# elybrand/quantized_neural_networks

Measured on NVIDIA B200. Metric: quantized weights/s, full-network GPFQ pass, higher is better.
Workload: dtype f64

## Files before the change

quantized_neural_networks_b200/csrc/api.cu:

```cuda
#include <math.h>
#include <stdarg.h>
#include <stdlib.h>

#include <algorithm>
#include <cmath>

#include "common.cuh"

int dense_gram_path(gpfq_ctx *, const float *, const float *, int64_t, int64_t, int64_t, const float *, int64_t,
                    int64_t, int64_t, const double *, const int *, const int *, int, double *, int64_t, int64_t,
                    gpfq_stats *, const double *G1_pre = nullptr, const double *G2_pre = nullptr, const double *d_scales = nullptr,
                    int64_t u0 = 0);
int dense_stream_path(gpfq_ctx *, const float *, const float *, int64_t, int64_t, int64_t, const float *, int64_t,
                      int64_t, int64_t, const double *, const int *, const int *, int, double *, int64_t, int64_t,
                      gpfq_stats *, const double *d_scales, int64_t u0);
int dense_gram_only(gpfq_ctx *, const float *, const float *, int64_t, int64_t, int64_t, double *, double *);
bool dense_gram_uses_i8(gpfq_ctx *, int64_t, int64_t, bool);
int conv_supported_kk(int kk);
int conv_pick_chunks(gpfq_ctx *, int64_t, int, int64_t *, int, bool, int64_t part_rows = 0);
bool conv_specialised_kk(int kk);
int conv_gram_stage(gpfq_ctx *, int, ConvPtrs, bool, int64_t, int, int, int64_t, double *, bool, int);
int conv_finalize_stage(gpfq_ctx *, const double *, int, int, int, bool, double *);
int conv_sweep_stage(gpfq_ctx *, int, const double *, const float *, double *, int64_t, int64_t, int64_t, int,
                     const double *, const int *, const int *, int, int64_t, const double *);
// ... 69 lines not shown
    *out = b.p;
    return GPFQ_OK;
}

extern "C" int gpfq_version(void) { return GPFQ_VERSION; }

extern "C" int gpfq_create(int device, gpfq_ctx **out) {
    if (!out) return GPFQ_ERR_ARG;
    *out = nullptr;
    int ndev = 0;
    if (cudaGetDeviceCount(&ndev) != cudaSuccess || device < 0 || device >= ndev) {
        cudaGetLastError();
        return GPFQ_ERR_UNSUPPORTED;
    }
    cudaDeviceProp prop;
    if (cudaGetDeviceProperties(&prop, device) != cudaSuccess) return GPFQ_ERR_CUDA;
    if (prop.major != 10) return GPFQ_ERR_UNSUPPORTED;
    if (cudaSetDevice(device) != cudaSuccess) return GPFQ_ERR_CUDA;
    gpfq_ctx *ctx = new gpfq_ctx();
    ctx->device = device;
    ctx->sm_count = prop.multiProcessorCount;
    ctx->smem_optin = prop.sharedMemPerBlockOptin;
    bool ok = cudaStreamCreateWithFlags(&ctx->own_stream, cudaStreamNonBlocking) == cudaSuccess &&
              cudaStreamCreateWithFlags(&ctx->copy_stream, cudaStreamNonBlocking) == cudaSuccess;
    ctx->ring.resize(GPFQ_RING);
    for (auto &r : ctx->ring)
        for (int i = 0; ok && i < 8; ++i) ok = cudaEventCreate(&r.e[i]) == cudaSuccess;
    ctx->cur = &ctx->ring[0];
    for (int i = 0; ok && i < 4; ++i) ok = cudaEventCreateWithFlags(&ctx->ev_copy[i], cudaEventDisableTiming) == cudaSuccess;
    for (int i = 0; ok && i < 12; ++i) ok = cudaEventCreateWithFlags(&ctx->ev_chain[i], cudaEventDisableTiming) == cudaSuccess;
    for (int i = 0; ok && i < 8; ++i) ok = cudaStreamCreateWithFlags(&ctx->aux_stream[i], cudaStreamNonBlocking) == cudaSuccess;
    if (!ok) {
        delete ctx;
        return GPFQ_ERR_CUDA;
    }
    ctx->stream = ctx->own_stream;
    *out = ctx;
    return GPFQ_OK;
}

extern "C" int64_t gpfq_conv_partial_bytes(gpfq_ctx *ctx) { return ctx ? ctx->conv_part_bytes : 0; }

extern "C" int gpfq_trim(gpfq_ctx *ctx) {
    if (!ctx) return GPFQ_ERR_ARG;
    cudaSetDevice(ctx->device);
    cudaStreamSynchronize(ctx->stream);
    cudaStreamSynchronize(ctx->copy_stream);
    for (auto &s : ctx->aux_stream) if (s) cudaStreamSynchronize(s);
    for (auto &b : ctx->ws) {
        if (b.p) cudaFree(b.p);
        b.p = nullptr;
        b.cap = 0;
    }
    for (auto &b : ctx->pinned) {
        if (b.p) cudaFreeHost(b.p);
        b.p = nullptr;
        b.cap = 0;
    }
    ctx->alph_cache.clear();
    ctx->alph_used = 0;
    ctx->i8_oom_bytes = 0;
    return GPFQ_OK;
}

extern "C" void gpfq_destroy(gpfq_ctx *ctx) {
    if (!ctx) return;
    gpfq_trim(ctx);
    for (auto &r : ctx->ring)
        for (auto &e : r.e) if (e) cudaEventDestroy(e);
    for (auto &e : ctx->ev_copy) if (e) cudaEventDestroy(e);
    for (auto &e : ctx->ev_chain) if (e) cudaEventDestroy(e);
    for (auto &s : ctx->aux_stream) if (s) cudaStreamDestroy(s);
    if (ctx->own_stream) cudaStreamDestroy(ctx->own_stream);
    if (ctx->copy_stream) cudaStreamDestroy(ctx->copy_stream);
    delete ctx;
}

extern "C" const char *gpfq_last_error(const gpfq_ctx *ctx) { return ctx ? ctx->err.c_str() : "null context"; }

extern "C" int gpfq_set_option(gpfq_ctx *ctx, const char *key, int64_t value) {
    if (!ctx || !key) return GPFQ_ERR_ARG;
    ctx->err.clear();
    if (!strcmp(key, "gram_kernel")) {
        if (value < 0 || value > 2) return gpfq_fail(ctx, GPFQ_ERR_ARG, "gram_kernel must be 0, 1 or 2");
        ctx->gram_variant = (int)value;
    } else if (!strcmp(key, "i8_pairs_d")) {
        if (value != 0 && (value < 2 || value > 10)) return gpfq_fail(ctx, GPFQ_ERR_ARG, "i8_pairs_d must be 0 or 2..10");
        ctx->i8_pairs_d = (int)value;
    } else if (!strcmp(key, "corr_pack")) {
        if (value < 0 || value > 2) return gpfq_fail(ctx, GPFQ_ERR_ARG, "corr_pack must be 0, 1 or 2");
        ctx->corr_pack = (int)value;
    } else if (!strcmp(key, "corr_small")) {
        ctx->corr_direct_small = value != 0;
    } else if (!strcmp(key, "corr_rows")) {
        if (value != 0 && value != 4 && value != 6 && value != 8) return gpfq_fail(ctx, GPFQ_ERR_ARG, "corr_rows must be 0, 4, 6 or 8");
        ctx->corr_rb = (int)value;
    } else if (!strcmp(key, "corr_strip")) {
        if (value != 0 && value != 2) return gpfq_fail(ctx, GPFQ_ERR_ARG, "corr_strip must be 0 or 2");
        ctx->corr_strip = (int)value;
    } else if (!strcmp(key, "conv_kernel")) {
        if (value < 0 || value > 3) return gpfq_fail(ctx, GPFQ_ERR_ARG, "conv_kernel must be 0, 1, 2 or 3");
        ctx->conv_variant = (int)value;
    } else if (!strcmp(key, "sweep_outer")) {
        if (value < 0 || value > 3) return gpfq_fail(ctx, GPFQ_ERR_ARG, "sweep_outer must be 0, 1, 2 or 3");
        ctx->lowrank_variant = (int)value;
    } else if (!strcmp(key, "sweep_walk")) {
        if (value < 0 || value > 2) return gpfq_fail(ctx, GPFQ_ERR_ARG, "sweep_walk must be 0, 1 or 2");
        ctx->sweep_walk = (int)value;
    } else if (!strcmp(key, "sweep_i8")) {
        if (value < 0 || value > 2) return gpfq_fail(ctx, GPFQ_ERR_ARG, "sweep_i8 must be 0, 1 or 2");
        ctx->sweep_i8 = (int)value;
    } else {
        return gpfq_fail(ctx, GPFQ_ERR_ARG, "unknown option '%s'", key);
    }
    return GPFQ_OK;
}

extern "C" int gpfq_set_rounding(gpfq_ctx *ctx, int32_t mode, const uint64_t *seeds, int32_t n_seeds) {
    if (!ctx) return GPFQ_ERR_ARG;
    ctx->err.clear();
    if (mode == GPFQ_ROUND_NEAREST) {
        ctx->rounding = mode;
        ctx->seeds.clear();
        return GPFQ_OK;
    }
    if (mode != GPFQ_ROUND_STOCHASTIC) return gpfq_fail(ctx, GPFQ_ERR_ARG, "unknown rounding mode %d", mode);
    if (!seeds || n_seeds < 1) return gpfq_fail(ctx, GPFQ_ERR_ARG, "stochastic rounding needs n_seeds >= 1 seeds");
    ctx->rounding = mode;
    ctx->seeds.assign(seeds, seeds + n_seeds);
    return GPFQ_OK;
}

extern "C" int gpfq_set_stream(gpfq_ctx *ctx, void *cuda_stream) {
    if (!ctx) return GPFQ_ERR_ARG;
    cudaStream_t next = cuda_stream ? (cudaStream_t)cuda_stream : ctx->own_stream;
    if (next != ctx->stream) {
        cudaSetDevice(ctx->device);
        if (cudaStreamSynchronize(ctx->stream) != cudaSuccess) cudaGetLastError();
        ctx->stream = next;
    }
    return GPFQ_OK;
}

struct Alphabets {
    const double *d_levels = nullptr;
    const int *d_koff = nullptr;
    const int *d_flags = nullptr;
    std::vector<int> h_koff, h_flags;
};

static int alphabet_is_equispaced(const double *a, int K) {
    if (K < 2) return 0;
    const double step = (a[K - 1] - a[0]) / (K - 1);
    if (!(step > 0.0) || !std::isfinite(step)) return 0;
    for (int k = 0; k < K; ++k)
        if (!(fabs(a[k] - (a[0] + k * step)) <= 0.01 * step)) return 0;
    return 1;
}

static int upload_alphabets(gpfq_ctx *ctx, const double *alphabets, const int32_t *K, int n_alph, Alphabets *out) {
    if (!alphabets || !K || n_alph < 1 || n_alph > 1024) return gpfq_fail(ctx, GPFQ_ERR_ARG, "bad alphabet arguments");
    out->h_koff.assign(n_alph + 1, 0);
    for (int a = 0; a < n_alph; ++a) {
        if (K[a] < 1 || K[a] > GPFQ_MAX_K)
// ... 1070 lines not shown
```

quantized_neural_networks_b200/csrc/common.cuh:

```cuda
#pragma once
#include <cuda_runtime.h>
#include <stdint.h>
#include <stdio.h>
#include <string.h>

#include <string>
#include <vector>

#include "../../include/gpfq.h"

#define GPFQ_DEAD_NORM 1e-16
#define GPFQ_PERP_DOT 1e-10

struct DevBuf {
    void *p = nullptr;
    size_t cap = 0;
};

struct ConvPtrs {
    const float *const *Xp;
    const float *const *Xqp;
};

struct AlphEntry {
    std::vector<char> blob;
    size_t off = 0;
};

struct CallRecord {
    cudaEvent_t e[8] = {};
    bool rec[8] = {};
    int kind = 0;
    gpfq_stats st = {};
};
static constexpr int GPFQ_RING = 128;

struct gpfq_ctx {
    int device = 0;
    int sm_count = 148;
    size_t smem_optin = 0;
    cudaStream_t own_stream = nullptr;
    cudaStream_t copy_stream = nullptr;
    cudaStream_t stream = nullptr;
    std::vector<CallRecord> ring;
    int64_t calls = 0;
    CallRecord *cur = nullptr;
    cudaEvent_t ev_copy[4] = {};
    cudaStream_t aux_stream[8] = {};
    cudaEvent_t ev_chain[12] = {};
    std::string err = "";
    int launches = 0;
    int conv_variant = 0;
    int corr_pack = 0;
    bool corr_direct_small = false;
    int corr_occ[2][9] = {};
    int corr_rb = 0;
    int corr_strip_occ[2][2][3] = {};
    int corr_strip = 0;
    bool stream_literal = false;
    int gram_variant = 0;
    int lowrank_variant = 0;
    int sweep_walk = 0;
    int sweep_i8 = 0;
    int i8_pairs_d = 0;
    const double *h_alph = nullptr;
    const int *h_koff = nullptr, *h_flags = nullptr;
    int64_t conv_part_bytes = 0;
    double *gram_only_out = nullptr;
    int last_gram_kernel = 0;
    size_t i8_oom_bytes = 0;
    int rounding = GPFQ_ROUND_NEAREST;
    std::vector<uint64_t> seeds;
    const uint64_t *d_seeds = nullptr;
    DevBuf ws[48];
    DevBuf pinned[4];
    std::vector<AlphEntry> alph_cache;
    size_t alph_used = 0;
};

enum WsSlot {
    WS_X = 0, WS_XQ, WS_W, WS_Q, WS_WT, WS_QT, WS_G1, WS_G2, WS_PART, WS_DT, WS_NRM, WS_ALPH,
    WS_U, WS_PTRS, WS_CG, WS_CPART, WS_PATCH_A, WS_PATCH_B, WS_ACT_A, WS_ACT_B, WS_QIDX, WS_MISC,
    WS_I8_SQ, WS_I8_SX, WS_I8_E, WS_I8_TILES, WS_LR_XD, WS_LR_XT, WS_LR_U, WS_CORR_B,
    WS_SL_W, WS_SL_XT, WS_SL_XQT, WS_SL_XQ, WS_SL_U, WS_SL_KQ, WS_SL_E,
    WS_TC_TAB, WS_TC_G2S, WS_TC_G1S, WS_TC_E, WS_TC_P, WS_TC_W, WS_TC_G1M, WS_SCALES, WS_UNIT_H, WS_SEEDS
};

int gpfq_fail(gpfq_ctx *ctx, int code, const char *fmt, ...);
cudaError_t gpfq_record(gpfq_ctx *ctx, int which, cudaStream_t s);
int gpfq_ws(gpfq_ctx *ctx, int slot, size_t bytes, void **out);
int gpfq_pinned(gpfq_ctx *ctx, int slot, size_t bytes, void **out);

#define CUDA_TRY(ctx, expr)                                                                    \
    do {                                                                                       \
        cudaError_t _e = (expr);                                                               \
        if (_e != cudaSuccess)                                                                 \
            return gpfq_fail((ctx), _e == cudaErrorMemoryAllocation ? GPFQ_ERR_OOM : GPFQ_ERR_CUDA, \
                             "%s failed: %s (%s:%d)", #expr, cudaGetErrorString(_e), __FILE__, __LINE__); \
    } while (0)

#define GPFQ_TRY(expr)                \
    do {                              \
        int _rc = (expr);             \
        if (_rc != GPFQ_OK) return _rc; \
    } while (0)

#define KERNEL_CHECK(ctx)                                                                     \
    do {                                                                                      \
        (ctx)->launches++;                                                                    \
        cudaError_t _e = cudaGetLastError();                                                  \
        if (_e != cudaSuccess)                                                                \
            return gpfq_fail((ctx), GPFQ_ERR_CUDA, "kernel launch failed: %s (%s:%d)",        \
                             cudaGetErrorString(_e), __FILE__, __LINE__);                     \
    } while (0)

static constexpr int64_t CONV_PART_LIMIT = (int64_t)1 << 30;

static inline int64_t ceil_div64(int64_t a, int64_t b) { return (a + b - 1) / b; }

__device__ __forceinline__ double gpfq_bit_round(double v, const double *__restrict__ alph, int K) {
    double best = alph[0];
    double bd = fabs(__dsub_rn(best, v));
#pragma unroll 4
    for (int k = 1; k < K; ++k) {
        const double a = alph[k];
        const double d = fabs(__dsub_rn(a, v));
        if (d < bd) { bd = d; best = a; }
// ... 178 lines not shown
```

quantized_neural_networks_b200/csrc/slgemm_i8.cu:

```cuda
#include <algorithm>

#include "slgemm_i8.cuh"

namespace slg {
constexpr int TM = 128, TN = 64, BK = 64;
constexpr int STAGES = 3;
constexpr int S = 5;
constexpr int P_BITS = 8 * S - 2;
constexpr int A_SLICE = TM * BK, B_SLICE = TN * BK;
constexpr int STAGE_BYTES = S * (A_SLICE + B_SLICE);
constexpr int THREADS = 192;
constexpr int MAX_PHASES = 8;
constexpr int OUT_PITCH = TN + 1;
constexpr int KB_MAX = 408;
constexpr size_t SMEM = (size_t)STAGES * STAGE_BYTES + 1024  + 256  + TN * sizeof(double);
}

struct SlSeg {
    int SA, SB, D;
    int a_row0, b_row0;
    int k0, k0b, kblocks;
    double alpha;
    const double *row_mul;
    const int32_t *eA;
    int eA_const;
    const int8_t *A, *B;
    int64_t rowsA, rowsB;
};

struct SlArgs {
    SlSeg seg[2];
    int nseg, tiles_n;
    const int32_t *eB;
    int eB_const, b_row0;
    double *C;
    int64_t ldc;
    int M, N;
    int accumulate, vec2;
    int batch_rows_a, batch_rows_b, batch_k0a, batch_k0b;
    int64_t batch_c;
    int lower_only;
    int ktri;
};

__device__ __forceinline__ uint64_t umma_desc_sw64(uint32_t saddr) {
    return (uint64_t)((saddr & 0x3FFFFu) >> 4) | ((uint64_t)1 << 16) | ((uint64_t)(512 >> 4) << 32) | ((uint64_t)1 << 46) |
           ((uint64_t)4 << 61);
}

template <int SA, int SB, int D>
__device__ __forceinline__ void sl_issue_kblock(uint32_t tmem_base, uint64_t da, uint64_t db, uint32_t idesc, bool first) {
    using namespace slg;
#pragma unroll
    for (int d = 2; d <= D; ++d) {
        constexpr int dummy = 0;
        (void)dummy;
        const int k_lo = (d - SB) > 1 ? (d - SB) : 1, k_hi = SA < (d - 1) ? SA : (d - 1);
#pragma unroll
        for (int k = k_lo; k <= k_hi; ++k)
#pragma unroll
            for (int ks = 0; ks < BK / 32; ++ks)
                i8g::umma_i8(tmem_base + (uint32_t)((d - 2) * TN), da + (uint64_t)(((k - 1) * A_SLICE + ks * 32) >> 4),
                             db + (uint64_t)(((d - k - 1) * B_SLICE + ks * 32) >> 4), idesc,
                             (k == k_lo && ks == 0) ? (first ? 0u : 1u) : 1u);
    }
}

template <bool ROWMUL>
__global__ void __launch_bounds__(slg::THREADS, 1)
slgemm_i8_kernel(const SlArgs args) {
    using namespace i8g;
    using namespace slg;
    extern __shared__ unsigned char sl_smem_raw[];
    unsigned char *smem = reinterpret_cast<unsigned char *>(((uintptr_t)sl_smem_raw + 1023) & ~(uintptr_t)1023);
    uint64_t *full = reinterpret_cast<uint64_t *>(smem + (size_t)STAGES * STAGE_BYTES);
    uint64_t *empty = full + STAGES;
    uint64_t *seg_full = empty + STAGES;
    uint64_t *seg_empty = seg_full + 1;
    uint32_t *tmem_slot = reinterpret_cast<uint32_t *>(seg_empty + 1);
    double *colscale = reinterpret_cast<double *>(smem + (size_t)STAGES * STAGE_BYTES + 256);

    const int warp = threadIdx.x >> 5, lane = threadIdx.x & 31;
    const int ti = blockIdx.x / args.tiles_n, tj = blockIdx.x % args.tiles_n;
    if (args.lower_only && tj * TN > ti * TM + TM - 1) return;
    const int brow_a = (int)blockIdx.y * args.batch_rows_a, brow_b = (int)blockIdx.y * args.batch_rows_b;
    const int bk0a = (int)blockIdx.y * args.batch_k0a, bk0b = (int)blockIdx.y * args.batch_k0b;
    const int kcap = args.ktri ? tj + 1 : (1 << 30);

    if (threadIdx.x == 0) {
        for (int s = 0; s < STAGES; ++s) { mbar_init(&full[s], 1); mbar_init(&empty[s], 1); }
        mbar_init(seg_full, 1);
        mbar_init(seg_empty, 4);
        asm volatile("fence.mbarrier_init.release.cluster;\n" ::: "memory");
    }
    if (warp == 1) {
        asm volatile("tcgen05.alloc.cta_group::1.sync.aligned.shared::cta.b32 [%0], %1;\n" ::"r"(smem_u32(tmem_slot)), "r"(512));
        asm volatile("tcgen05.relinquish_alloc_permit.cta_group::1.sync.aligned;\n");
    }
    if (warp >= 2 && threadIdx.x - 64 < TN) {
        const int c = threadIdx.x - 64;
        colscale[c] = ldexp(1.0, args.eB ? args.eB[args.b_row0 + brow_b + tj * TN + c] : args.eB_const);
    }
    asm volatile("tcgen05.fence::before_thread_sync;\n" ::: "memory");
    __syncthreads();
    asm volatile("tcgen05.fence::after_thread_sync;\n" ::: "memory");
    const uint32_t tmem_base = *tmem_slot;

    if (warp == 0) {
        if (lane == 0) {
            int iter = 0;
            for (int sg = 0; sg < args.nseg; ++sg) {
                const SlSeg &g = args.seg[sg];
                const uint32_t bytes = (uint32_t)(g.SA * A_SLICE + g.SB * B_SLICE);
                const int8_t *pa = g.A + ((int64_t)((g.k0 + bk0a) / BK) * g.SA * g.rowsA + g.a_row0 + brow_a + ti * TM) * BK;
                const int8_t *pb = g.B + ((int64_t)((g.k0b + bk0b) / BK) * g.SB * g.rowsB + g.b_row0 + brow_b + tj * TN) * BK;
                const int kblocks = min(g.kblocks, kcap);
                const int64_t a_slice = g.rowsA * BK, b_slice = g.rowsB * BK;
                for (int kb = 0; kb < kblocks; ++kb, ++iter) {
                    const int s = iter % STAGES;
                    if (iter >= STAGES) mbar_wait(&empty[s], ((iter / STAGES) - 1) & 1);
                    unsigned char *a = smem + (size_t)s * STAGE_BYTES, *b = a + S * A_SLICE;
                    mbar_expect_tx(&full[s], bytes);
                    for (int sl = 0; sl < g.SA; ++sl) bulk_load(a + sl * A_SLICE, pa + ((int64_t)kb * g.SA + sl) * a_slice, A_SLICE, &full[s]);
                    for (int sl = 0; sl < g.SB; ++sl) bulk_load(b + sl * B_SLICE, pb + ((int64_t)kb * g.SB + sl) * b_slice, B_SLICE, &full[s]);
                }
            }
        }
    } else if (warp == 1) {
        {
            const uint32_t idesc = (2u << 4) | (1u << 7) | (1u << 10) | ((uint32_t)(TN >> 3) << 17) | ((uint32_t)(TM >> 4) << 24);
            int iter = 0;
            for (int sg = 0; sg < args.nseg; ++sg) {
                const SlSeg &g = args.seg[sg];
                if (sg > 0) {
                    mbar_wait(seg_empty, (sg - 1) & 1);
                    asm volatile("tcgen05.fence::after_thread_sync;\n" ::: "memory");
                }
                const int mode = (g.SA == 5 && g.SB == 5 && g.D == 6) ? 1 : (g.SA == 5 && g.SB == 5 && g.D == 7) ? 2
                                 : (g.SA == 1 && g.SB == 5 && g.D == 6) ? 3 : 0;
                const int kblocks = min(g.kblocks, kcap);
                for (int kb = 0; kb < kblocks; ++kb, ++iter) {
                    const int s = iter % STAGES;
                    mbar_wait(&full[s], (iter / STAGES) & 1);
                    asm volatile("tcgen05.fence::after_thread_sync;\n" ::: "memory");
                    const uint32_t a = smem_u32(smem + (size_t)s * STAGE_BYTES), b = a + S * A_SLICE;
                    const uint64_t da = umma_desc_sw64(a), db = umma_desc_sw64(b);
                    if (elect_one()) {
                        if (mode == 1) sl_issue_kblock<5, 5, 6>(tmem_base, da, db, idesc, kb == 0);
                        else if (mode == 2) sl_issue_kblock<5, 5, 7>(tmem_base, da, db, idesc, kb == 0);
                        else if (mode == 3) sl_issue_kblock<1, 5, 6>(tmem_base, da, db, idesc, kb == 0);
                        else
                            for (int d = 2; d <= g.D; ++d) {
                                const uint32_t tmem_d = tmem_base + (uint32_t)((d - 2) * TN);
                                const int k_lo = max(1, d - g.SB), k_hi = min(g.SA, d - 1);
                                for (int k = k_lo; k <= k_hi; ++k) {
                                    const uint32_t ak = a + (k - 1) * A_SLICE, bl = b + (d - k - 1) * B_SLICE;
#pragma unroll
                                    for (int ks = 0; ks < BK / 32; ++ks)
                                        umma_i8(tmem_d, umma_desc_sw64(ak + ks * 32), umma_desc_sw64(bl + ks * 32), idesc,
                                                (kb | (k - k_lo) | ks) ? 1u : 0u);
                                }
                            }
                        umma_commit(&empty[s]);
                    }
                    __syncwarp();
                }
                if (elect_one()) umma_commit(seg_full);
                __syncwarp();
            }
        }
    } else {
        const int quad = warp & 3;
        const int row_t = quad * 32 + lane;
        const uint32_t lane_field = (uint32_t)(quad * 32) << 16;
        double acc[TN];
#pragma unroll
        for (int i = 0; i < TN; ++i) acc[i] = 0.0;
        for (int sg = 0; sg < args.nseg; ++sg) {
            const SlSeg &g = args.seg[sg];
            const int ea = g.eA ? g.eA[g.a_row0 + brow_a + ti * TM + row_t] : g.eA_const;
            const double alpha = (ROWMUL && g.row_mul) ? g.alpha * g.row_mul[g.a_row0 + brow_a + ti * TM + row_t] : g.alpha;
            mbar_wait(seg_full, sg & 1);
            asm volatile("tcgen05.fence::after_thread_sync;\n" ::: "memory");
#pragma unroll 1
            for (int d = 2; d <= g.D; ++d) {
                const double rs = ldexp(alpha, 4 - 8 * d + ea);
#pragma unroll
                for (int hf = 0; hf < TN / 32; ++hf) {
                    uint32_t v[32];
                    tmem_ld32(tmem_base + lane_field + (uint32_t)((d - 2) * TN + hf * 32), v);
#pragma unroll
                    for (int i = 0; i < 32; ++i) acc[hf * 32 + i] = fma((double)(int)v[i], rs, acc[hf * 32 + i]);
                }
            }
            asm volatile("tcgen05.fence::before_thread_sync;\n" ::: "memory");
            __syncwarp();
            if (lane == 0) mbar_arrive(seg_empty);
        }
        double *tr = reinterpret_cast<double *>(smem) + (size_t)quad * 32 * OUT_PITCH;
#pragma unroll
        for (int i = 0; i < TN; ++i) tr[lane * OUT_PITCH + i] = acc[i] * colscale[i];
        __syncwarp();
        const int64_t row0 = (int64_t)ti * TM + quad * 32, col0 = (int64_t)tj * TN;
        double *Cb = args.C + (int64_t)blockIdx.y * args.batch_c;
        double old[32][TN / 32];
#pragma unroll
        for (int r = 0; r < 32; ++r)
#pragma unroll
            for (int hf = 0; hf < TN / 32; ++hf) {
                const int c = hf * 32 + lane;
                old[r][hf] = (args.accumulate && row0 + r < args.M && col0 + c < args.N) ? Cb[(row0 + r) * args.ldc + col0 + c] : 0.0;
            }
#pragma unroll
        for (int r = 0; r < 32; ++r)
#pragma unroll
            for (int hf = 0; hf < TN / 32; ++hf) {
                const int c = hf * 32 + lane;
                if (row0 + r < args.M && col0 + c < args.N) Cb[(row0 + r) * args.ldc + col0 + c] = old[r][hf] + tr[r * OUT_PITCH + c];
            }
    }
    asm volatile("tcgen05.fence::before_thread_sync;\n" ::: "memory");
    __syncthreads();
    if (warp == 1) {
        asm volatile("tcgen05.fence::after_thread_sync;\n" ::: "memory");
        asm volatile("tcgen05.dealloc.cta_group::1.sync.aligned.b32 %0, %1;\n" ::"r"(tmem_base), "r"(512));
    }
}

template <typename T>
__global__ void __launch_bounds__(256) sl_rowsplit_kernel(const T *__restrict__ X, int64_t ldx, int64_t rows, int64_t cols,
                                                          int32_t *__restrict__ e, int8_t *__restrict__ slices, int64_t rowsP,
                                                          int64_t colsP, int64_t row0) {
    using namespace slg;
    __shared__ double red[8];
    __shared__ int ex_s;
    const int64_t r = blockIdx.x;
    const T *row = X + r * ldx;
    double mx = 0.0;
    if (r < rows)
        for (int64_t i = threadIdx.x; i < cols; i += 256) mx = fmax(mx, fabs((double)row[i]));
#pragma unroll
    for (int o = 16; o > 0; o >>= 1) mx = fmax(mx, __shfl_xor_sync(0xffffffffu, mx, o));
    if ((threadIdx.x & 31) == 0) red[threadIdx.x >> 5] = mx;
    __syncthreads();
    if (threadIdx.x == 0) {
        for (int w = 1; w < 8; ++w) mx = fmax(mx, red[w]);
        int ex = 0;
        if (mx > 0.0 && isfinite(mx)) frexp(mx, &ex);
        e[row0 + r] = ex;
        ex_s = ex;
    }
    __syncthreads();
    const int ex = ex_s;
    for (int64_t i0 = (int64_t)threadIdx.x * 16; i0 < colsP; i0 += 256 * 16) {
        uint32_t packed[S][4];
#pragma unroll
        for (int k = 0; k < S; ++k) packed[k][0] = packed[k][1] = packed[k][2] = packed[k][3] = 0u;
        if (r < rows && i0 < cols) {
#pragma unroll
            for (int c = 0; c < 16; ++c) {
                const double x = (i0 + c < cols) ? (double)row[i0 + c] : 0.0;
                long long v = __double2ll_rn(ldexp(x, P_BITS - ex));
#pragma unroll
                for (int k = S - 1; k >= 0; --k) {
                    const int dg = (int)((v + 128) & 255) - 128;
                    v = (v - dg) >> 8;
                    packed[k][c >> 2] |= ((uint32_t)(dg & 0xff)) << (8 * (c & 3));
                }
            }
        }
#pragma unroll
        for (int k = 0; k < S; ++k)
// ... 141 lines not shown
    if (nprod < 1 || nprod > 2) return gpfq_fail(ctx, GPFQ_ERR_ARG, "slgemm_i8: 1 or 2 products");
    SlArgs a = {};
    a.nseg = nprod;
    for (int s = 0; s < nprod; ++s) {
        const SlProduct &p = prod[s];
        const int64_t k0b = p.k0b < 0 ? p.k0 : p.k0b;
        if (p.K % BK || p.k0 % BK || k0b % BK || batch.a_k % BK || batch.b_k % BK || p.K / BK > KB_MAX || p.K < BK)
            return gpfq_fail(ctx, GPFQ_ERR_ARG, "slgemm_i8: K = %lld (offset %lld) must be multiples of 64, at most %d",
                             (long long)p.K, (long long)p.k0, KB_MAX * BK);
        if (p.A->is_b || !p.B->is_b || p.A->n_slices > S || p.B->n_slices > S)
            return gpfq_fail(ctx, GPFQ_ERR_ARG, "slgemm_i8: operand roles / slice counts");
        if (p.a_row0 + (nbatch - 1) * batch.a_rows + ceil_div64(M, TM) * TM > p.A->rowsP ||
            p.b_row0 + (nbatch - 1) * batch.b_rows + ceil_div64(N, TN) * TN > p.B->rowsP ||
            p.k0 + (nbatch - 1) * batch.a_k + p.K > p.A->kbytes || k0b + (nbatch - 1) * batch.b_k + p.K > p.B->kbytes)
            return gpfq_fail(ctx, GPFQ_ERR_ARG, "slgemm_i8: operand slices are not padded to the tile grid");
        if (s > 0 && (p.B->e != prod[0].B->e || p.B->e_const != prod[0].B->e_const || p.b_row0 != prod[0].b_row0))
            return gpfq_fail(ctx, GPFQ_ERR_ARG, "slgemm_i8: the products of one call must share the exponents of their B rows");
        SlSeg &g = a.seg[s];
        g.SA = p.A->n_slices;
        g.SB = p.B->n_slices;
        g.D = std::min(std::min(p.D, g.SA + g.SB), MAX_PHASES + 1);
        g.a_row0 = (int)p.a_row0;
        g.b_row0 = (int)p.b_row0;
        g.k0 = (int)p.k0;
        g.k0b = (int)k0b;
        g.kblocks = (int)(p.K / BK);
        g.alpha = p.alpha;
        g.row_mul = p.row_mul;
        g.eA = p.A->e;
        g.eA_const = p.A->e_const;
        g.A = p.A->slices;
        g.B = p.B->slices;
        g.rowsA = p.A->rowsP;
        g.rowsB = p.B->rowsP;
    }
    a.eB = prod[0].B->e;
    a.eB_const = prod[0].B->e_const;
    a.b_row0 = (int)prod[0].b_row0;
    a.tiles_n = (int)ceil_div64(N, TN);
    a.C = C;
    a.ldc = ldc;
    a.M = (int)M;
    a.N = (int)N;
    a.accumulate = accumulate ? 1 : 0;
    a.vec2 = (ldc % 2 == 0) && ((uintptr_t)C % 16 == 0);
    a.batch_rows_a = (int)batch.a_rows;
    a.batch_rows_b = (int)batch.b_rows;
    a.batch_k0a = (int)batch.a_k;
    a.batch_k0b = (int)batch.b_k;
    a.batch_c = batch.c;
    a.lower_only = batch.lower_only ? 1 : 0;
    a.ktri = batch.ktri ? 1 : 0;
    if (nbatch < 1 || nbatch > 65535) return gpfq_fail(ctx, GPFQ_ERR_ARG, "slgemm_i8: 1..65535 batches");
    const bool rowmul = a.seg[0].row_mul || (nprod > 1 && a.seg[1].row_mul);
    auto k = rowmul ? slgemm_i8_kernel<true> : slgemm_i8_kernel<false>;
    CUDA_TRY(ctx, cudaFuncSetAttribute(k, cudaFuncAttributeMaxDynamicSharedMemorySize, (int)SMEM));
    const dim3 grid((unsigned)(ceil_div64(M, TM) * a.tiles_n), (unsigned)nbatch);
    k<<<grid, THREADS, SMEM, ctx->stream>>>(a);
    KERNEL_CHECK(ctx);
    return GPFQ_OK;
}

template <typename T>
int sl_rowsplit(gpfq_ctx *ctx, const T *X, int64_t ldx, int64_t rows, int64_t cols, int32_t *e, int8_t *slices, int64_t rowsP,
                int64_t colsP, int64_t row0, int64_t grid_rows) {
    const unsigned wgrid = (unsigned)ceil_div64(grid_rows, 8);
    if (colsP <= 32 * 16 * 2)
        sl_rowsplit_warp_kernel<T, 2><<<wgrid, 256, 0, ctx->stream>>>(X, ldx, rows, cols, e, slices, rowsP, colsP, row0, grid_rows);
    else if (colsP <= 32 * 16 * 4)
        sl_rowsplit_warp_kernel<T, 4><<<wgrid, 256, 0, ctx->stream>>>(X, ldx, rows, cols, e, slices, rowsP, colsP, row0, grid_rows);
    else
        sl_rowsplit_kernel<T><<<(unsigned)grid_rows, 256, 0, ctx->stream>>>(X, ldx, rows, cols, e, slices, rowsP, colsP, row0);
    KERNEL_CHECK(ctx);
    return GPFQ_OK;
}
template int sl_rowsplit<double>(gpfq_ctx *, const double *, int64_t, int64_t, int64_t, int32_t *, int8_t *, int64_t, int64_t, int64_t, int64_t);
template int sl_rowsplit<float>(gpfq_ctx *, const float *, int64_t, int64_t, int64_t, int32_t *, int8_t *, int64_t, int64_t, int64_t, int64_t);

int sl_transsplit(gpfq_ctx *ctx, const float *X, const float *Xq, int64_t ldx, int64_t N0, int64_t m, int32_t *e, int *scratch,
                  int8_t *slices, int8_t *slices_q, int64_t mP, int64_t N0P) {
    cudaStream_t st = ctx->stream;
    CUDA_TRY(ctx, cudaMemsetAsync(scratch, 0, (size_t)mP * sizeof(int), st));
    const int rows_per_cta = 256;
    dim3 g1((unsigned)ceil_div64(m, 256), (unsigned)ceil_div64(N0, rows_per_cta));
    sl_colmax_kernel<<<g1, 256, 0, st>>>(X, ldx, N0, m, scratch, rows_per_cta);
    KERNEL_CHECK(ctx);
    if (Xq) {
        sl_colmax_kernel<<<g1, 256, 0, st>>>(Xq, ldx, N0, m, scratch, rows_per_cta);
        KERNEL_CHECK(ctx);
    }
    sl_exp_from_max_kernel<<<(unsigned)ceil_div64(mP, 256), 256, 0, st>>>(scratch, m, mP, e);
    KERNEL_CHECK(ctx);
    dim3 g2((unsigned)(N0P / 64), (unsigned)(mP / 32));
    sl_transsplit_kernel<<<g2, 128, 0, st>>>(X, ldx, N0, m, e, slices, mP, N0P);
    KERNEL_CHECK(ctx);
    if (Xq) {
        sl_transsplit_kernel<<<g2, 128, 0, st>>>(Xq, ldx, N0, m, e, slices_q, mP, N0P);
        KERNEL_CHECK(ctx);
    }
    return GPFQ_OK;
}

extern "C" int gpfq_debug_slgemm(gpfq_ctx *ctx, const double *A, const float *B, int64_t M, int64_t N, int64_t K, int32_t D,
                                 int32_t transposed_b, double *C_out) {
    using namespace slg;
    if (!ctx) return GPFQ_ERR_ARG;
    ctx->err.clear();
    if (!A || !B || !C_out || M < 1 || N < 1 || K < 1) return gpfq_fail(ctx, GPFQ_ERR_ARG, "bad arguments");
    CUDA_TRY(ctx, cudaSetDevice(ctx->device));
    cudaStream_t st = ctx->stream;
// ... 33 lines not shown
```

Baseline: 2.136 billion.

## Add split-K and persistent tile scheduling to int8 sliced GEMM kernel

Reworks the tcgen05 sliced int8 GEMM so each CTA walks a list of work units (batch, tile, K-split) instead of one tile per block. It adds optional split-K, where partial integer accumulators go to a global workspace and the last CTA to arrive reduces them through a ticket counter. The epilogue is restructured into a per-half transpose that is used when a CTA has more units queued. Both split-K and the grid cap are off by default (split=0, grid=units), so the default path differs only in the flattened 1-D grid, the unit decoding and the column-scale reads moving from shared memory into per-lane registers.

```diff
diff --git a/quantized_neural_networks_b200/csrc/api.cu b/quantized_neural_networks_b200/csrc/api.cu
--- a/quantized_neural_networks_b200/csrc/api.cu
+++ b/quantized_neural_networks_b200/csrc/api.cu
@@ -145,6 +145,11 @@
         b.p = nullptr;
         b.cap = 0;
     }
+    for (auto &w : ctx->split_ws) {
+        if (w.part.p) cudaFree(w.part.p);
+        if (w.cnt.p) cudaFree(w.cnt.p);
+    }
+    ctx->split_ws.clear();
     for (auto &b : ctx->pinned) {
         if (b.p) cudaFreeHost(b.p);
         b.p = nullptr;
@@ -203,6 +208,12 @@
     } else if (!strcmp(key, "sweep_i8")) {
         if (value < 0 || value > 2) return gpfq_fail(ctx, GPFQ_ERR_ARG, "sweep_i8 must be 0, 1 or 2");
         ctx->sweep_i8 = (int)value;
+    } else if (!strcmp(key, "slgemm_split")) {
+        if (value < 0 || value > 8) return gpfq_fail(ctx, GPFQ_ERR_ARG, "slgemm_split must be 0..8");
+        ctx->slgemm_split = (int)value;
+    } else if (!strcmp(key, "slgemm_grid")) {
+        if (value < 0 || value > 65535) return gpfq_fail(ctx, GPFQ_ERR_ARG, "slgemm_grid must be 0..65535");
+        ctx->slgemm_grid = (int)value;
     } else {
         return gpfq_fail(ctx, GPFQ_ERR_ARG, "unknown option '%s'", key);
     }
diff --git a/quantized_neural_networks_b200/csrc/common.cuh b/quantized_neural_networks_b200/csrc/common.cuh
--- a/quantized_neural_networks_b200/csrc/common.cuh
+++ b/quantized_neural_networks_b200/csrc/common.cuh
@@ -63,6 +63,8 @@
     int sweep_walk = 0;
     int sweep_i8 = 0;
     int i8_pairs_d = 0;
+    int slgemm_split = 0;
+    int slgemm_grid = 0;
     const double *h_alph = nullptr;
     const int *h_koff = nullptr, *h_flags = nullptr;
     int64_t conv_part_bytes = 0;
@@ -73,6 +75,8 @@
     std::vector<uint64_t> seeds;
     const uint64_t *d_seeds = nullptr;
     DevBuf ws[48];
+    struct SplitWs { cudaStream_t s; DevBuf part, cnt; };
+    std::vector<SplitWs> split_ws;
     DevBuf pinned[4];
     std::vector<AlphEntry> alph_cache;
     size_t alph_used = 0;
diff --git a/quantized_neural_networks_b200/csrc/slgemm_i8.cu b/quantized_neural_networks_b200/csrc/slgemm_i8.cu
--- a/quantized_neural_networks_b200/csrc/slgemm_i8.cu
+++ b/quantized_neural_networks_b200/csrc/slgemm_i8.cu
@@ -11,9 +11,11 @@
 constexpr int STAGE_BYTES = S * (A_SLICE + B_SLICE);
 constexpr int THREADS = 192;
 constexpr int MAX_PHASES = 8;
-constexpr int OUT_PITCH = TN + 1;
+constexpr int TR_PITCH = 33;
+constexpr int TR_BYTES = 4 * 32 * TR_PITCH * (int)sizeof(double);
 constexpr int KB_MAX = 408;
-constexpr size_t SMEM = (size_t)STAGES * STAGE_BYTES + 1024  + 256  + TN * sizeof(double);
+constexpr int MAX_SPLIT = 8;
+constexpr size_t SMEM = (size_t)STAGES * STAGE_BYTES + 1024  + 256  + TR_BYTES;
 }
 
 struct SlSeg {
@@ -41,7 +43,38 @@
     int64_t batch_c;
     int lower_only;
     int ktri;
+    int tiles_m, units;
+    int ks, nacc;
+    int32_t *part;
+    int *cnt;
 };
+
+__device__ __forceinline__ bool sl_unit(const SlArgs &a, int u, int &bt, int &ti, int &tj, int &sp) {
+    using namespace slg;
+    sp = u % a.ks;
+    int t = u / a.ks;
+    const int tiles = a.tiles_m * a.tiles_n;
+    bt = t / tiles;
+    t -= bt * tiles;
+    ti = t / a.tiles_n;
+    tj = t - ti * a.tiles_n;
+    return !(a.lower_only && tj * TN > ti * TM + TM - 1);
+}
+
+__device__ __forceinline__ int sl_next_unit(const SlArgs &a, int u) {
+    int bt, ti, tj, sp;
+    for (u += gridDim.x; u < a.units; u += gridDim.x)
+        if (sl_unit(a, u, bt, ti, tj, sp)) break;
+    return u < a.units ? u : a.units;
+}
+
+__device__ __forceinline__ void sl_krange(const SlArgs &a, const SlSeg &g, int tj, int sp, int &kb0, int &kb1) {
+    const int kb = min(g.kblocks, a.ktri ? tj + 1 : (1 << 30));
+    kb0 = sp * kb / a.ks;
+    kb1 = (sp + 1) * kb / a.ks;
+}
+
+__device__ __forceinline__ void sl_epi_bar() { asm volatile("bar.sync 1, 128;\n" ::: "memory"); }
 
 __device__ __forceinline__ uint64_t umma_desc_sw64(uint32_t saddr) {
     return (uint64_t)((saddr & 0x3FFFFu) >> 4) | ((uint64_t)1 << 16) | ((uint64_t)(512 >> 4) << 32) | ((uint64_t)1 << 46) |
@@ -78,14 +111,10 @@
     uint64_t *seg_full = empty + STAGES;
     uint64_t *seg_empty = seg_full + 1;
     uint32_t *tmem_slot = reinterpret_cast<uint32_t *>(seg_empty + 1);
-    double *colscale = reinterpret_cast<double *>(smem + (size_t)STAGES * STAGE_BYTES + 256);
+    volatile int *ticket_s = reinterpret_cast<volatile int *>(tmem_slot + 1);
+    double *trans = reinterpret_cast<double *>(smem + (size_t)STAGES * STAGE_BYTES + 256);
 
     const int warp = threadIdx.x >> 5, lane = threadIdx.x & 31;
-    const int ti = blockIdx.x / args.tiles_n, tj = blockIdx.x % args.tiles_n;
-    if (args.lower_only && tj * TN > ti * TM + TM - 1) return;
-    const int brow_a = (int)blockIdx.y * args.batch_rows_a, brow_b = (int)blockIdx.y * args.batch_rows_b;
-    const int bk0a = (int)blockIdx.y * args.batch_k0a, bk0b = (int)blockIdx.y * args.batch_k0b;
-    const int kcap = args.ktri ? tj + 1 : (1 << 30);
 
     if (threadIdx.x == 0) {
         for (int s = 0; s < STAGES; ++s) { mbar_init(&full[s], 1); mbar_init(&empty[s], 1); }
@@ -97,10 +126,6 @@
         asm volatile("tcgen05.alloc.cta_group::1.sync.aligned.shared::cta.b32 [%0], %1;\n" ::"r"(smem_u32(tmem_slot)), "r"(512));
         asm volatile("tcgen05.relinquish_alloc_permit.cta_group::1.sync.aligned;\n");
     }
-    if (warp >= 2 && threadIdx.x - 64 < TN) {
-        const int c = threadIdx.x - 64;
-        colscale[c] = ldexp(1.0, args.eB ? args.eB[args.b_row0 + brow_b + tj * TN + c] : args.eB_const);
-    }
     asm volatile("tcgen05.fence::before_thread_sync;\n" ::: "memory");
     __syncthreads();
     asm volatile("tcgen05.fence::after_thread_sync;\n" ::: "memory");
@@ -109,46 +134,57 @@
     if (warp == 0) {
         if (lane == 0) {
             int iter = 0;
-            for (int sg = 0; sg < args.nseg; ++sg) {
-                const SlSeg &g = args.seg[sg];
-                const uint32_t bytes = (uint32_t)(g.SA * A_SLICE + g.SB * B_SLICE);
-                const int8_t *pa = g.A + ((int64_t)((g.k0 + bk0a) / BK) * g.SA * g.rowsA + g.a_row0 + brow_a + ti * TM) * BK;
-                const int8_t *pb = g.B + ((int64_t)((g.k0b + bk0b) / BK) * g.SB * g.rowsB + g.b_row0 + brow_b + tj * TN) * BK;
-                const int kblocks = min(g.kblocks, kcap);
-                const int64_t a_slice = g.rowsA * BK, b_slice = g.rowsB * BK;
-                for (int kb = 0; kb < kblocks; ++kb, ++iter) {
-                    const int s = iter % STAGES;
-                    if (iter >= STAGES) mbar_wait(&empty[s], ((iter / STAGES) - 1) & 1);
-                    unsigned char *a = smem + (size_t)s * STAGE_BYTES, *b = a + S * A_SLICE;
-                    mbar_expect_tx(&full[s], bytes);
-                    for (int sl = 0; sl < g.SA; ++sl) bulk_load(a + sl * A_SLICE, pa + ((int64_t)kb * g.SA + sl) * a_slice, A_SLICE, &full[s]);
-                    for (int sl = 0; sl < g.SB; ++sl) bulk_load(b + sl * B_SLICE, pb + ((int64_t)kb * g.SB + sl) * b_slice, B_SLICE, &full[s]);
+            for (int u = blockIdx.x; u < args.units; u += gridDim.x) {
+                int bt, ti, tj, sp;
+                if (!sl_unit(args, u, bt, ti, tj, sp)) continue;
+                const int brow_a = bt * args.batch_rows_a, brow_b = bt * args.batch_rows_b;
+                const int bk0a = bt * args.batch_k0a, bk0b = bt * args.batch_k0b;
+                for (int sg = 0; sg < args.nseg; ++sg) {
+                    const SlSeg &g = args.seg[sg];
+                    const uint32_t bytes = (uint32_t)(g.SA * A_SLICE + g.SB * B_SLICE);
+                    const int8_t *pa = g.A + ((int64_t)((g.k0 + bk0a) / BK) * g.SA * g.rowsA + g.a_row0 + brow_a + ti * TM) * BK;
+                    const int8_t *pb = g.B + ((int64_t)((g.k0b + bk0b) / BK) * g.SB * g.rowsB + g.b_row0 + brow_b + tj * TN) * BK;
+                    int kb0, kb1;
+                    sl_krange(args, g, tj, sp, kb0, kb1);
+                    const int64_t a_slice = g.rowsA * BK, b_slice = g.rowsB * BK;
+                    for (int kb = kb0; kb < kb1; ++kb, ++iter) {
+                        const int s = iter % STAGES;
+                        if (iter >= STAGES) mbar_wait(&empty[s], ((iter / STAGES) - 1) & 1);
+                        unsigned char *a = smem + (size_t)s * STAGE_BYTES, *b = a + S * A_SLICE;
+                        mbar_expect_tx(&full[s], bytes);
+                        for (int sl = 0; sl < g.SA; ++sl) bulk_load(a + sl * A_SLICE, pa + ((int64_t)kb * g.SA + sl) * a_slice, A_SLICE, &full[s]);
+                        for (int sl = 0; sl < g.SB; ++sl) bulk_load(b + sl * B_SLICE, pb + ((int64_t)kb * g.SB + sl) * b_slice, B_SLICE, &full[s]);
+                    }
                 }
             }
         }
     } else if (warp == 1) {
-        {
-            const uint32_t idesc = (2u << 4) | (1u << 7) | (1u << 10) | ((uint32_t)(TN >> 3) << 17) | ((uint32_t)(TM >> 4) << 24);
-            int iter = 0;
-            for (int sg = 0; sg < args.nseg; ++sg) {
+        const uint32_t idesc = (2u << 4) | (1u << 7) | (1u << 10) | ((uint32_t)(TN >> 3) << 17) | ((uint32_t)(TM >> 4) << 24);
+        int iter = 0, sc = 0;
+        for (int u = blockIdx.x; u < args.units; u += gridDim.x) {
+            int bt, ti, tj, sp;
+            if (!sl_unit(args, u, bt, ti, tj, sp)) continue;
+            for (int sg = 0; sg < args.nseg; ++sg, ++sc) {
                 const SlSeg &g = args.seg[sg];
-                if (sg > 0) {
-                    mbar_wait(seg_empty, (sg - 1) & 1);
+                if (sc > 0) {
+                    mbar_wait(seg_empty, (sc - 1) & 1);
                     asm volatile("tcgen05.fence::after_thread_sync;\n" ::: "memory");
                 }
                 const int mode = (g.SA == 5 && g.SB == 5 && g.D == 6) ? 1 : (g.SA == 5 && g.SB == 5 && g.D == 7) ? 2
                                  : (g.SA == 1 && g.SB == 5 && g.D == 6) ? 3 : 0;
-                const int kblocks = min(g.kblocks, kcap);
-                for (int kb = 0; kb < kblocks; ++kb, ++iter) {
+                int kb0, kb1;
+                sl_krange(args, g, tj, sp, kb0, kb1);
+                for (int kb = kb0; kb < kb1; ++kb, ++iter) {
                     const int s = iter % STAGES;
                     mbar_wait(&full[s], (iter / STAGES) & 1);
                     asm volatile("tcgen05.fence::after_thread_sync;\n" ::: "memory");
                     const uint32_t a = smem_u32(smem + (size_t)s * STAGE_BYTES), b = a + S * A_SLICE;
                     const uint64_t da = umma_desc_sw64(a), db = umma_desc_sw64(b);
+                    const bool first = kb == kb0;
                     if (elect_one()) {
-                        if (mode == 1) sl_issue_kblock<5, 5, 6>(tmem_base, da, db, idesc, kb == 0);
-                        else if (mode == 2) sl_issue_kblock<5, 5, 7>(tmem_base, da, db, idesc, kb == 0);
-                        else if (mode == 3) sl_issue_kblock<1, 5, 6>(tmem_base, da, db, idesc, kb == 0);
+                        if (mode == 1) sl_issue_kblock<5, 5, 6>(tmem_base, da, db, idesc, first);
+                        else if (mode == 2) sl_issue_kblock<5, 5, 7>(tmem_base, da, db, idesc, first);
+                        else if (mode == 3) sl_issue_kblock<1, 5, 6>(tmem_base, da, db, idesc, first);
                         else
                             for (int d = 2; d <= g.D; ++d) {
                                 const uint32_t tmem_d = tmem_base + (uint32_t)((d - 2) * TN);
@@ -158,7 +194,7 @@
 #pragma unroll
                                     for (int ks = 0; ks < BK / 32; ++ks)
                                         umma_i8(tmem_d, umma_desc_sw64(ak + ks * 32), umma_desc_sw64(bl + ks * 32), idesc,
-                                                (kb | (k - k_lo) | ks) ? 1u : 0u);
+                                                (!first || (k - k_lo) | ks) ? 1u : 0u);
                                 }
                             }
                         umma_commit(&empty[s]);
@@ -173,51 +209,134 @@
         const int quad = warp & 3;
         const int row_t = quad * 32 + lane;
         const uint32_t lane_field = (uint32_t)(quad * 32) << 16;
-        double acc[TN];
-#pragma unroll
-        for (int i = 0; i < TN; ++i) acc[i] = 0.0;
-        for (int sg = 0; sg < args.nseg; ++sg) {
-            const SlSeg &g = args.seg[sg];
-            const int ea = g.eA ? g.eA[g.a_row0 + brow_a + ti * TM + row_t] : g.eA_const;
-            const double alpha = (ROWMUL && g.row_mul) ? g.alpha * g.row_mul[g.a_row0 + brow_a + ti * TM + row_t] : g.alpha;
-            mbar_wait(seg_full, sg & 1);
-            asm volatile("tcgen05.fence::after_thread_sync;\n" ::: "memory");
+        double *tr = trans + (size_t)quad * 32 * TR_PITCH;
+        const int npart = args.ks - 1;
+        int sc = 0;
+        for (int u = blockIdx.x; u < args.units; u += gridDim.x) {
+            int bt, ti, tj, sp;
+            if (!sl_unit(args, u, bt, ti, tj, sp)) continue;
+            const int brow_a = bt * args.batch_rows_a, brow_b = bt * args.batch_rows_b;
+            const int tile = u / args.ks;
+            double acc[TN];
+#pragma unroll
+            for (int i = 0; i < TN; ++i) acc[i] = 0.0;
+            bool partial = false;
+            double cs[TN / 32];
+#pragma unroll
+            for (int hf = 0; hf < TN / 32; ++hf)
+                cs[hf] = ldexp(1.0, args.eB ? args.eB[args.b_row0 + brow_b + tj * TN + hf * 32 + lane] : args.eB_const);
+            for (int sg = 0; sg < args.nseg; ++sg, ++sc) {
+                const SlSeg &g = args.seg[sg];
+                const int ea = g.eA ? g.eA[g.a_row0 + brow_a + ti * TM + row_t] : g.eA_const;
+                const double alpha = (ROWMUL && g.row_mul) ? g.alpha * g.row_mul[g.a_row0 + brow_a + ti * TM + row_t] : g.alpha;
+                mbar_wait(seg_full, sc & 1);
+                asm volatile("tcgen05.fence::after_thread_sync;\n" ::: "memory");
+                if (npart > 0) {
+                    int *cnt = args.cnt + 2 * (int64_t)tile;
+                    if (threadIdx.x == 64) *ticket_s = atomicAdd(cnt, 1);
+                    sl_epi_bar();
+                    const int ticket = *ticket_s;
+                    if (ticket < npart) {
+                        int32_t *dst = args.part + ((int64_t)tile * npart + ticket) * args.nacc * (TM * TN) + row_t;
 #pragma unroll 1
-            for (int d = 2; d <= g.D; ++d) {
-                const double rs = ldexp(alpha, 4 - 8 * d + ea);
-#pragma unroll
-                for (int hf = 0; hf < TN / 32; ++hf) {
-                    uint32_t v[32];
-                    tmem_ld32(tmem_base + lane_field + (uint32_t)((d - 2) * TN + hf * 32), v);
-#pragma unroll
-                    for (int i = 0; i < 32; ++i) acc[hf * 32 + i] = fma((double)(int)v[i], rs, acc[hf * 32 + i]);
+                        for (int d = 2; d <= g.D; ++d)
+#pragma unroll
+                            for (int hf = 0; hf < TN / 32; ++hf) {
+                                uint32_t v[32];
+                                tmem_ld32(tmem_base + lane_field + (uint32_t)((d - 2) * TN + hf * 32), v);
+#pragma unroll
+                                for (int i = 0; i < 32; ++i) __stcg(dst + ((d - 2) * TN + hf * 32 + i) * TM, (int)v[i]);
+                            }
+                        asm volatile("tcgen05.fence::before_thread_sync;\n" ::: "memory");
+                        __syncwarp();
+                        if (lane == 0) mbar_arrive(seg_empty);
+                        __threadfence();
+                        sl_epi_bar();
+                        if (threadIdx.x == 64) {
+                            __threadfence();
+                            atomicAdd(cnt + 1, 1);
+                        }
+                        partial = true;
+                        continue;
+                    }
+                    if (threadIdx.x == 64) {
+                        int done;
+                        for (;;) {
+                            asm volatile("ld.acquire.gpu.global.b32 %0, [%1];\n" : "=r"(done) : "l"(cnt + 1) : "memory");
+                            if (done >= npart) break;
+                            __nanosleep(64);
+                        }
+                        cnt[0] = 0;
+                        cnt[1] = 0;
+                    }
+                    sl_epi_bar();
+                    __threadfence();
                 }
+                const int32_t *src = args.part + (int64_t)tile * npart * args.nacc * (TM * TN) + row_t;
+#pragma unroll 1
+                for (int d = 2; d <= g.D; ++d) {
+                    const double rs = ldexp(alpha, 4 - 8 * d + ea);
+#pragma unroll
+                    for (int hf = 0; hf < TN / 32; ++hf) {
+                        uint32_t v[32];
+                        tmem_ld32(tmem_base + lane_field + (uint32_t)((d - 2) * TN + hf * 32), v);
+                        if (npart > 0)
+#pragma unroll 1
+                            for (int p = 0; p < npart; ++p)
+#pragma unroll
+                                for (int i = 0; i < 32; ++i)
+                                    v[i] += (uint32_t)__ldcg(src + ((int64_t)(p * args.nacc + d - 2) * TN + hf * 32 + i) * TM);
+#pragma unroll
+                        for (int i = 0; i < 32; ++i) acc[hf * 32 + i] = fma((double)(int)v[i], rs, acc[hf * 32 + i]);
+                    }
+                }
+                asm volatile("tcgen05.fence::before_thread_sync;\n" ::: "memory");
+                __syncwarp();
+                if (lane == 0) mbar_arrive(seg_empty);
             }
-            asm volatile("tcgen05.fence::before_thread_sync;\n" ::: "memory");
-            __syncwarp();
-            if (lane == 0) mbar_arrive(seg_empty);
-        }
-        double *tr = reinterpret_cast<double *>(smem) + (size_t)quad * 32 * OUT_PITCH;
-#pragma unroll
-        for (int i = 0; i < TN; ++i) tr[lane * OUT_PITCH + i] = acc[i] * colscale[i];
-        __syncwarp();
-        const int64_t row0 = (int64_t)ti * TM + quad * 32, col0 = (int64_t)tj * TN;
-        double *Cb = args.C + (int64_t)blockIdx.y * args.batch_c;
-        double old[32][TN / 32];
-#pragma unroll
-        for (int r = 0; r < 32; ++r)
+            if (partial) continue;
+            const int64_t row0 = (int64_t)ti * TM + quad * 32, col0 = (int64_t)tj * TN;
+            double *Cb = args.C + (int64_t)bt * args.batch_c;
+            if (sl_next_unit(args, u) >= args.units) {
+                double *tw = reinterpret_cast<double *>(smem) + (size_t)quad * 32 * (TN + 1);
+#pragma unroll
+                for (int i = 0; i < TN; ++i) tw[lane * (TN + 1) + i] = acc[i];
+                __syncwarp();
+                double old[32][TN / 32];
+#pragma unroll
+                for (int r = 0; r < 32; ++r)
+#pragma unroll
+                    for (int hf = 0; hf < TN / 32; ++hf) {
+                        const int c = hf * 32 + lane;
+                        old[r][hf] = (args.accumulate && row0 + r < args.M && col0 + c < args.N) ? Cb[(row0 + r) * args.ldc + col0 + c] : 0.0;
+                    }
+#pragma unroll
+                for (int r = 0; r < 32; ++r)
+#pragma unroll
+                    for (int hf = 0; hf < TN / 32; ++hf) {
+                        const int c = hf * 32 + lane;
+                        if (row0 + r < args.M && col0 + c < args.N)
+                            Cb[(row0 + r) * args.ldc + col0 + c] = old[r][hf] + __dmul_rn(tw[r * (TN + 1) + c], cs[hf]);
+                    }
+                continue;
+            }
 #pragma unroll
             for (int hf = 0; hf < TN / 32; ++hf) {
                 const int c = hf * 32 + lane;
-                old[r][hf] = (args.accumulate && row0 + r < args.M && col0 + c < args.N) ? Cb[(row0 + r) * args.ldc + col0 + c] : 0.0;
+#pragma unroll
+                for (int i = 0; i < 32; ++i) tr[lane * TR_PITCH + i] = acc[hf * 32 + i];
+                __syncwarp();
+                double old[32];
+#pragma unroll
+                for (int r = 0; r < 32; ++r)
+                    old[r] = (args.accumulate && row0 + r < args.M && col0 + c < args.N) ? Cb[(row0 + r) * args.ldc + col0 + c] : 0.0;
+#pragma unroll
+                for (int r = 0; r < 32; ++r)
+                    if (row0 + r < args.M && col0 + c < args.N)
+                        Cb[(row0 + r) * args.ldc + col0 + c] = old[r] + __dmul_rn(tr[r * TR_PITCH + lane], cs[hf]);
+                __syncwarp();
             }
-#pragma unroll
-        for (int r = 0; r < 32; ++r)
-#pragma unroll
-            for (int hf = 0; hf < TN / 32; ++hf) {
-                const int c = hf * 32 + lane;
-                if (row0 + r < args.M && col0 + c < args.N) Cb[(row0 + r) * args.ldc + col0 + c] = old[r][hf] + tr[r * OUT_PITCH + c];
-            }
+        }
     }
     asm volatile("tcgen05.fence::before_thread_sync;\n" ::: "memory");
     __syncthreads();
@@ -465,10 +584,45 @@
     a.lower_only = batch.lower_only ? 1 : 0;
     a.ktri = batch.ktri ? 1 : 0;
     if (nbatch < 1 || nbatch > 65535) return gpfq_fail(ctx, GPFQ_ERR_ARG, "slgemm_i8: 1..65535 batches");
+    a.tiles_m = (int)ceil_div64(M, TM);
+    const int64_t tiles = (int64_t)a.tiles_m * a.tiles_n * nbatch;
+    int ks = 1;
+    if (nprod == 1 && !batch.ktri && ctx->slgemm_split > 1) ks = std::min(ctx->slgemm_split, std::min(a.seg[0].kblocks, MAX_SPLIT));
+    if (tiles * ks > INT32_MAX) return gpfq_fail(ctx, GPFQ_ERR_ARG, "slgemm_i8: too many tiles");
+    a.ks = ks;
+    a.units = (int)(tiles * ks);
+    a.nacc = a.seg[0].D - 1;
+    if (ks > 1) {
+        gpfq_ctx::SplitWs *w = nullptr;
+        for (auto &x : ctx->split_ws)
+            if (x.s == ctx->stream) w = &x;
+        if (!w) {
+            ctx->split_ws.push_back({ctx->stream, {}, {}});
+            w = &ctx->split_ws.back();
+        }
+        const size_t part_bytes = (size_t)tiles * (ks - 1) * a.nacc * TM * TN * sizeof(int32_t), cnt_bytes = (size_t)tiles * 2 * sizeof(int);
+        for (int which = 0; which < 2; ++which) {
+            DevBuf &buf = which ? w->cnt : w->part;
+            const size_t bytes = which ? cnt_bytes : part_bytes;
+            if (buf.cap >= bytes) continue;
+            if (buf.p) {
+                CUDA_TRY(ctx, cudaStreamSynchronize(ctx->stream));
+                CUDA_TRY(ctx, cudaFree(buf.p));
+                buf.p = nullptr;
+                buf.cap = 0;
+            }
+            const size_t cap = (bytes + ((size_t)1 << 20) - 1) & ~(((size_t)1 << 20) - 1);
+            CUDA_TRY(ctx, cudaMalloc(&buf.p, cap));
+            buf.cap = cap;
+            if (which) CUDA_TRY(ctx, cudaMemsetAsync(buf.p, 0, cap, ctx->stream));
+        }
+        a.part = reinterpret_cast<int32_t *>(w->part.p);
+        a.cnt = reinterpret_cast<int *>(w->cnt.p);
+    }
     const bool rowmul = a.seg[0].row_mul || (nprod > 1 && a.seg[1].row_mul);
     auto k = rowmul ? slgemm_i8_kernel<true> : slgemm_i8_kernel<false>;
     CUDA_TRY(ctx, cudaFuncSetAttribute(k, cudaFuncAttributeMaxDynamicSharedMemorySize, (int)SMEM));
-    const dim3 grid((unsigned)(ceil_div64(M, TM) * a.tiles_n), (unsigned)nbatch);
+    const int grid = (int)std::min<int64_t>(a.units, ctx->slgemm_grid > 0 ? ctx->slgemm_grid : a.units);
     k<<<grid, THREADS, SMEM, ctx->stream>>>(a);
     KERNEL_CHECK(ctx);
     return GPFQ_OK;
```

New measurement: 2.152 billion, median of 6. No clear change (+0.8%).
